# yanqinJiang/Animate3D

Hardware: AMD Instinct MI355X
Metric: UNet denoise-steps/sec, 4view×16frame×512² MV-VDM @1/2/4/8 GPU (higher is better)
Workload: dtype bf16; 1 GPU; BASELINE config 2: 4 views x 16 frames x 512^2 px (64x64 latent), CFG-doubled batch V=8 videos, one MVUNetMotionModel.forward per step, SD1.5 MV-VDM UNet 1.53 B params, seeded synthetic weights; parallelism=single GPU

## Files before the change

### animate3d_amd/csrc/flash_attn.hip

```cpp
#include <type_traits>
#include <utility>

#include "common.h"
#include "flash_common.h"


namespace {

template <int D, int BKV, int QT, int OFS, bool ALIGNED, bool TWO = false>
__global__ __launch_bounds__(256, 2) void flash_attn_kernel(const AttnParams p) {
  constexpr int NU = BKV / 32;
  constexpr int VROW = BKV + 8;
  constexpr int DK = (D + 15) / 16 * 16;
  constexpr int KS = DK / 16;
  constexpr int MT = (D + 31) / 32;
  constexpr int KROW = DK + 8;
  constexpr int DCH = D / 8;
  constexpr int KCHUNKS = BKV * DCH;
  constexpr int KPT = (KCHUNKS + 255) / 256;
  constexpr int VITEMS = (BKV / 4) * DCH;
  constexpr int VPT = (VITEMS + 255) / 256;
  constexpr bool ONES = MT * 32 > D;
  constexpr int KS_ELEMS = BKV * KROW, VT_ELEMS = MT * 32 * VROW;
  constexpr int BQW = 32 * QT, BQ = 4 * BQW;
// ... 455 lines not shown
                     int groups, int heads, int head_dim, int64_t q_len, int64_t kv_len, int64_t kv_len2,
                     float scale, float out_scale, float out_scale2, int flags, int allowed, AttnParams& p, bool& aligned) {
  if (!Q || !K || !V || !O || groups <= 0 || heads <= 0 || q_len <= 0 || kv_len <= 0) return A3D_EINVAL;
  if (two && (!K2 || !V2 || kv_len2 <= 0)) return A3D_EINVAL;
  if (!map_ok(qmap, head_dim) || !map_ok(kmap, head_dim) || (two && !map_ok(kmap2, head_dim)) || !map_ok(omap, head_dim)) return A3D_EINVAL;
  if (!a3d_aligned(16, Q, K, V, K2, V2) || !a3d_aligned(8, O)) return A3D_EINVAL;
  if (groups > 65535 || q_len > 0x3fffffffLL || kv_len > 0x3fffffffLL || kmap->seg_len > 0x3fffffffLL) return A3D_EINVAL;
  if (two && (kv_len2 > 0x3fffffffLL || kmap2->seg_len > 0x3fffffffLL)) return A3D_EINVAL;
  if (two && head_dim != 40 && head_dim != 80) return A3D_EUNSUPPORTED;
  if (flags & ~allowed) return A3D_EINVAL;
  p = AttnParams{};
  p.Q = (const uint16_t*)Q; p.K = (const uint16_t*)K; p.V = (const uint16_t*)V; p.O = (uint16_t*)O;
  p.qm = *qmap; p.km = *kmap; p.om = *omap;
  p.heads = heads; p.q_len = (int)q_len; p.kv_len = (int)kv_len;
  p.scale_log2 = scale * 1.4426950408889634f; p.out_scale = out_scale;
  p.accumulate = flags & A3D_ATTN_ACCUMULATE; p.causal = (flags & A3D_ATTN_CAUSAL) != 0;
  if (p.causal && head_dim != 64 && head_dim != 160) return A3D_EUNSUPPORTED;
  const int bkv = head_dim == 160 ? 32 : 64;
  aligned = (kmap->seg_len % bkv == 0) || (kv_len <= kmap->seg_len);
  if (two) {
    p.K2 = (const uint16_t*)K2; p.V2 = (const uint16_t*)V2; p.km2 = *kmap2; p.kv_len2 = (int)kv_len2; p.out_scale2 = out_scale2;
    aligned = aligned && ((kmap2->seg_len % bkv == 0) || (kv_len2 <= kmap2->seg_len));
  }
  return A3D_OK;
}

static int flash_attn_impl(a3d_stream_t stream, const void* Q, const void* K, const void* V, void* O,
                           const a3d_rowmap* qmap, const a3d_rowmap* kmap, const a3d_rowmap* omap,
                           int groups, int heads, int head_dim, int64_t q_len, int64_t kv_len,
                           float scale, float out_scale, int accumulate, float* lse, unsigned int* counters = nullptr) {
  AttnParams p;
  bool aligned;
  if (int rc = attn_args(false, Q, K, V, nullptr, nullptr, O, qmap, kmap, nullptr, omap, groups, heads, head_dim, q_len, kv_len, 0,
                         scale, out_scale, 0.f, accumulate, A3D_ATTN_ACCUMULATE | A3D_ATTN_CAUSAL | A3D_ATTN_EXACT | A3D_ATTN_PLAIN, p, aligned)) return rc;
  const bool exact = (accumulate & A3D_ATTN_EXACT) != 0, plain = (accumulate & A3D_ATTN_PLAIN) != 0;
  p.lse = lse;
  p.counters = counters;
  hipStream_t s = (hipStream_t)stream;
  switch (head_dim) {
    case 40:
      if (q_len <= 128) { launch<40, 64, 1, OFS_PAD>(aligned, groups, s, p); break; }
      if (!plain && aligned && kv_len % 64 == 0 && kv_len >= 256 && q_len >= 256) {
        if (int rc = A3D_FN(a3d_launch_flash_dm)(exact ? 4 : 5, groups, s, p)) return rc;
        break;
      }
      launch<40, 64, 2, OFS_PAD>(aligned, groups, s, p);
      break;
    case 80:
      if (!plain && aligned && kv_len % 64 == 0 && kv_len >= 512 && q_len >= 256) {
        if (int rc = A3D_FN(a3d_launch_flash_dm80)(exact ? 0 : 1, groups, s, p)) return rc;
        break;
      }
      if (q_len >= 2048 && kv_len >= 2048) { launch<80, 32, 2, OFS_FMA>(aligned, groups, s, p); break; }
      launch<80, 64, 1, OFS_ACC>(aligned, groups, s, p);
      break;
    case 64: launch<64, 64, 1, OFS_FMA>(aligned, groups, s, p); break;
    case 160:
      if (!plain && !p.causal && kv_len % 64 == 0 && kv_len >= 256 && ((kmap->seg_len % 64 == 0) || (kv_len <= kmap->seg_len)) &&
          a3d_aligned(16, O) && omap->ld % 8 == 0) {
        if (int rc = A3D_FN(a3d_launch_flash_dm160)(exact ? 0 : 1, groups, s, p)) return rc;
        break;
      }
      launch<160, 32, 1, OFS_FMA>(aligned, groups, s, p);
      break;
    default: return A3D_EUNSUPPORTED;
  }
  return a3d_launch_status();
}
// ... 42 lines not shown
```

### animate3d_amd/csrc/flash_attn_dm80.hip

```cpp
#include "flash_common.h"

namespace {

constexpr int E_ROWB = 160;
constexpr int E_UNITB = 32 * E_ROWB;
constexpr int E_KB = 2 * E_UNITB;
constexpr int E_TILEB = 2 * E_KB;
constexpr int E_RING = 5;
constexpr int E_CV = E_RING * E_TILEB + 32;
constexpr int E_CV_BYTES = 2752;
constexpr int E_SAMPLE = E_CV + E_CV_BYTES;
constexpr int E_SMEM_BYTES = E_SAMPLE + E_UNITB;
constexpr float E_L_BAD = 1.2676506e30f;
#ifdef A3D_STORAGE_F16
constexpr float E_BIAS = F16_BIAS;
constexpr bool E_SAMPLED = true;
#else
constexpr float E_BIAS = 40.f;
constexpr bool E_SAMPLED = false;
#endif

extern __shared__ __attribute__((aligned(16))) uint8_t e_smem[];
A3D_DEV u32x4_t e_lds128(uint32_t off) { return *reinterpret_cast<const u32x4_t*>(e_smem + off); }
A3D_DEV u32x2_t e_ldstr(uint32_t off) { return lds_tr16_b64(reinterpret_cast<const uint16_t*>(e_smem + off)); }

template <int FLAGS>
__global__ __launch_bounds__(512, 2) void flash_attn_dm80_kernel(const AttnParams p) {
  constexpr int D = 80, KS = 5, MT = 3, NT = 512, BQ = 256;
  constexpr int NEXP = 16, NCVT = 8, NDMA = 3;
  constexpr bool TRY_NOMAX = (FLAGS & 1) != 0;

  const int tid = threadIdx.x, lane = tid & 63, wid = tid >> 6;
  const int w = __builtin_amdgcn_readfirstlane(wid);
  const int l31 = lane & 31, g = lane >> 5, i16 = lane & 15, q4 = lane >> 4;
  const int head = blockIdx.x % p.heads;
  const int qt = blockIdx.x / p.heads;
  const int64_t grp = blockIdx.y;
  const int64_t hoff = (int64_t)head * D;
  const uint32_t lds0 = fa_lds_addr(e_smem);

  for (int i = tid; i < E_CV_BYTES / 2; i += NT) {
    const int vb = 2 * i;
    reinterpret_cast<uint16_t*>(e_smem + E_CV)[i] = (vb == 0 || vb == 160 || vb == 2560 || vb == 2720) ? ONE16 : (uint16_t)0;
  }

  const int64_t ld = p.km.ld;
  const int64_t kgbase = map_group_base(p.km, grp);
  const uint32_t seg_len = (uint32_t)p.km.seg_len;
  const int64_t tile_step = (int64_t)64 * ld;
  const int64_t wrap_step = (p.km.seg_stride - p.km.seg_len) * ld;
  auto slot_src = [&](int slot) -> uint32_t {
    const bool isk = slot < 640;
    const int s2 = isk ? slot : slot - 640;
    const int prow = s2 / 10, cpos = s2 % 10;
    const int c = isk ? (cpos ^ ((prow >> 3) & 1)) : cpos;
    const int key = isk ? prow : ((prow & ~7) | (((prow & 7) >> 1) + 4 * (prow & 1)));
    return (uint32_t)(((int64_t)key * ld + c * 8) * 2);
  };
  const uint32_t voffA = slot_src(64 * w + lane);
  const uint32_t voffB = slot_src(512 + 64 * w + lane);
  const uint32_t voffC = slot_src(1024 + 32 * w + l31);
  uint32_t voffS = 0;
  if constexpr (E_SAMPLED) {
    const int ss = (64 * w + lane) % 320, prow = ss / 10;
    const int64_t key = (int64_t)prow * (p.kv_len / 32);
    voffS = (uint32_t)((map_seq(p.km, key) * ld + ((ss % 10) ^ ((prow >> 3) & 1)) * 8) * 2);
  }
  const uint64_t maskS = w < 5 ? ~0ull : 0ull;

  const int krow = kperm(l31);
  const uint32_t klane = (uint32_t)(krow * E_ROWB + 16 * (g ^ ((krow >> 3) & 1)));
  const int c4 = i16 & 3;
  const uint32_t vrow = (uint32_t)((8 * (q4 >> 1) + 2 * (i16 >> 2)) * E_ROWB);
  const uint32_t vlane01 = vrow + (uint32_t)(2 * (16 * (q4 & 1) + 4 * c4));
  const bool v2_data = (q4 & 1) == 0;
  const uint32_t vlane2 = v2_data ? vrow + (uint32_t)(2 * (64 + 4 * c4)) : (c4 == 0 ? (uint32_t)E_CV : (uint32_t)(E_CV + 8));
  uint32_t vmul = v2_data ? 1u : 0u;
  asm volatile("" : "+v"(vmul));

  const uint16_t* gA = nullptr;
  const uint16_t* gB = nullptr;
  const uint16_t* gC = nullptr;
  uint32_t seg_off = 0;
  auto dma_reset = [&]() __attribute__((always_inline)) {
    gA = dm_scalar(p.K + hoff + kgbase * ld);
    gB = dm_scalar((w < 2 ? p.K : p.V) + hoff + kgbase * ld);
    gC = dm_scalar(p.V + hoff + kgbase * ld);
    seg_off = 0;
  };
  auto tile_base = [&](int tile) __attribute__((always_inline)) -> uint32_t { return (uint32_t)((tile % E_RING) * E_TILEB); };
  auto dma_a = [&](int tile) __attribute__((always_inline)) { dm_glds16(voffA, gA, lds0 + tile_base(tile) + 1024 * w); };
  auto dma_b = [&](int tile) __attribute__((always_inline)) { dm_glds16(voffB, gB, lds0 + tile_base(tile) + 8192 + 1024 * w); };
  auto dma_c = [&](int tile) __attribute__((always_inline)) {
    dm_glds16_m(voffC, gC, lds0 + tile_base(tile) + 16384 + 512 * w, 0xffffffffull);
    seg_off += 64;
    int64_t stp = tile_step;
    if (seg_off >= seg_len) { stp += wrap_step; seg_off = 0; }
    gA += stp; gB += stp; gC += stp;
  };
  auto prologue_issue = [&]() __attribute__((always_inline)) {
    dma_reset();
    if constexpr (E_SAMPLED && TRY_NOMAX)
      dm_glds16_m(voffS, dm_scalar(p.K + hoff + kgbase * ld), lds0 + (uint32_t)(E_SAMPLE + 1024 * (w < 5 ? w : 0)), maskS);
    dma_a(0); dma_b(0); dma_c(0);
    dma_a(1); dma_b(1); dma_c(1);
    dma_a(2); dma_b(2); dma_c(2);
  };
  auto prologue_wait = [&]() __attribute__((always_inline)) { asm volatile("s_waitcnt vmcnt(%0)\n\ts_barrier" :: "i"(NDMA) : "memory"); };
  prologue_issue();

  const int q_idx = qt * BQ + wid * 32 + l31;
  u32x4_t qf[KS];
  {
    const int64_t q_row = map_row(p.qm, grp, q_idx < p.q_len ? q_idx : p.q_len - 1);
#pragma unroll
    for (int ks = 0; ks < KS; ++ks) {
      u32x4_t wq = *reinterpret_cast<const u32x4_t*>(p.Q + q_row * p.qm.ld + hoff + 16 * ks + 8 * g);
#pragma unroll
      for (int j = 0; j < 4; ++j) wq[j] = pack16(lo16(wq[j]) * p.scale_log2, hi16(wq[j]) * p.scale_log2);
      qf[ks] = wq;
    }
  }


  f32x16_t oacc[MT];
  f32x16_t minit;
  u32x4_t kf[KS];
  u32x4_t vf[MT][2];
  auto read_k = [&](uint32_t koff) __attribute__((always_inline)) {
    const uint32_t a = klane + koff;
#pragma unroll
    for (int ks = 0; ks < KS; ++ks) kf[ks] = e_lds128(a + 32 * ks);
  };
  auto read_vhalf = [&](auto i_c, uint32_t a01, uint32_t a2) __attribute__((always_inline)) {
    constexpr int i = decltype(i_c)::value, h = i / 6, mt = (i / 2) % 3, rr = i % 2;
    const u32x2_t t = e_ldstr((mt == 2 ? a2 : a01 + 64 * mt) + (16 * h + rr) * E_ROWB);
    vf[mt][h][2 * rr] = t[0];
    vf[mt][h][2 * rr + 1] = t[1];
  };
  auto read_v = [&](uint32_t voff) __attribute__((always_inline)) {
    const uint32_t a01 = vlane01 + voff, a2 = __umul24(vmul, voff) + vlane2;
    static_for<12>([&](auto i_c) __attribute__((always_inline)) { read_vhalf(i_c, a01, a2); });
  };
  auto pv_mfma = [&](auto i_c, u32x4_t (&P)[2]) __attribute__((always_inline)) {
    constexpr int i = decltype(i_c)::value, h = i / 3, mt = i % 3;
    oacc[mt] = mfma32(vf[mt][h], P[h], oacc[mt]);
  };
  auto clear_o = [&]() __attribute__((always_inline)) {
#pragma unroll
    for (int mt = 0; mt < MT; ++mt)
#pragma unroll
      for (int r = 0; r < 16; ++r) oacc[mt][r] = 0.f;
#pragma unroll
    for (int r = 0; r < 16; ++r) minit[r] = 0.f;
  };
  const int nt = p.kv_len / 64;
  auto first_scores = [&](f32x16_t& s, float& m_off, float bias, uint32_t koff = 0u) __attribute__((always_inline)) -> bool {
    read_k(koff);
#pragma unroll
    for (int r = 0; r < 16; ++r) s[r] = 0.f;
#pragma unroll
    for (int ks = 0; ks < KS; ++ks) s = mfma32(kf[ks], qf[ks], s);
    float mx = s[0];
#pragma unroll
    for (int r = 1; r < 16; ++r) mx = fmaxf(mx, s[r]);
    mx = fmaxf(mx, __shfl_xor(mx, 32));
    bool wide = false;
    if constexpr (E_SAMPLED) {
      if (bias != 0.f) {
        float sm = 0.f, sq = 0.f;
#pragma unroll
        for (int r = 0; r < 16; ++r) { sm += s[r]; sq = fmaf(s[r], s[r], sq); }
        sm += __shfl_xor(sm, 32); sq += __shfl_xor(sq, 32);
        const float mean = sm * (1.f / 32.f);
        bias = f16_sampled_bias(mx, mean, sq * (1.f / 32.f) - mean * mean, f16_expected_max_sds(p.kv_len), wide);
      }
    }
    m_off = mx + bias;
#pragma unroll
    for (int r = 0; r < 16; ++r) { s[r] -= m_off; minit[r] = -m_off; }
    return wide;
  };
  auto finish = [&](bool check) __attribute__((always_inline)) -> bool {
    const float l_tot = __shfl(oacc[2][8], l31);
    const bool bad = !(l_tot < E_L_BAD) || !(l_tot > 0.f);
    if (check) {
      if (__syncthreads_or(bad ? 1 : 0)) { dm_count(p, 1); return false; }
    }
    const float inv = p.out_scale / l_tot;
    if (p.lse != nullptr && q_idx < p.q_len && g == 0)
// ... 13 lines not shown
              const uint32_t w0 = pack16(oacc[mt][8 * pr + 2 * c] * inv, oacc[mt][8 * pr + 2 * c + 1] * inv);
              const uint32_t w1 = pack16(oacc[mt][8 * pr + 4 + 2 * c] * inv, oacc[mt][8 * pr + 4 + 2 * c + 1] * inv);
              const auto r = __builtin_amdgcn_permlane32_swap(w0, w1, false, false);
              v[c] = r[0];
              v[2 + c] = r[1];
            }
            *reinterpret_cast<u32x4_t*>(orow + 32 * mt + 16 * pr + 8 * g) = v;
          }
      } else {
#pragma unroll
        for (int mt = 0; mt < MT; ++mt)
#pragma unroll
          for (int qd = 0; qd < 4; ++qd) {
            const int d = 32 * mt + 8 * qd + 4 * g;
            if (d < D) {
              float v[4];
#pragma unroll
              for (int j = 0; j < 4; ++j) v[j] = oacc[mt][4 * qd + j] * inv;
              if (p.accumulate) {
                const u32x2_t prev = *reinterpret_cast<const u32x2_t*>(orow + d);
                v[0] += lo16(prev[0]); v[1] += hi16(prev[0]); v[2] += lo16(prev[1]); v[3] += hi16(prev[1]);
              }
              u32x2_t o;
              o[0] = pack16(v[0], v[1]);
              o[1] = pack16(v[2], v[3]);
              *reinterpret_cast<u32x2_t*>(orow + d) = o;
            }
          }
      }
    }
    return true;
  };

  auto run_fast = [&]() __attribute__((always_inline)) -> bool {
    clear_o();
    f32x16_t sA, sB;
    u32x4_t pA[2], pB[2];
#pragma unroll
    for (int h = 0; h < 2; ++h) { pA[h] = u32x4_t{0u, 0u, 0u, 0u}; pB[h] = u32x4_t{0u, 0u, 0u, 0u}; }

    auto step = [&](auto do_qk_c, auto do_pv_c, f32x16_t& sCur, f32x16_t& sNext, u32x4_t (&pCur)[2], u32x4_t (&pPrev)[2],
                    uint32_t kOff, uint32_t vOff, auto&& hook) __attribute__((always_inline)) {
      constexpr bool DO_QK = decltype(do_qk_c)::value, DO_PV = decltype(do_pv_c)::value;
      constexpr int NPV = DO_PV ? 2 * MT : 0, NQK = DO_QK ? KS : 0, NS = NPV + NQK;
      constexpr int KSLOT = 2, VS0 = NPV + 1, VPS = 3;
      const uint32_t va01 = vlane01 + vOff, va2 = __umul24(vmul, vOff) + vlane2;
      float e[NEXP];
      auto do_cvt = [&](auto c_c) __attribute__((always_inline)) {
        constexpr int c = decltype(c_c)::value, h = c / 4, jj = c % 4;
        pCur[h][jj] = pack16(e[2 * c], e[2 * c + 1]);
      };
      auto cdone = [](int s) constexpr { return s < 0 ? 0 : (NEXP * s / NS) / 2; };
      __builtin_amdgcn_sched_barrier(0);
      static_for<NS>([&](auto s_c) __attribute__((always_inline)) {
        constexpr int s = decltype(s_c)::value;
        if constexpr (s < NPV) {
          pv_mfma(s_c, pPrev);
        } else {
          constexpr int ks = s - NPV;
          if constexpr (ks == 0) sNext = mfma32(kf[0], qf[0], minit);
          else sNext = mfma32(kf[ks], qf[ks], sNext);
        }
        if constexpr (DO_QK && DO_PV && s == KSLOT) read_k(kOff);
        if constexpr (DO_QK && s >= VS0 && VPS * (s - VS0) < 12) {
          static_for<VPS>([&](auto i_c) __attribute__((always_inline)) {
            constexpr int i = VPS * (s - VS0) + decltype(i_c)::value;
            if constexpr (i < 12) read_vhalf(std::integral_constant<int, i>{}, va01, va2);
          });
        }
        hook(s_c);
        constexpr int E0 = NEXP * s / NS, E1 = NEXP * (s + 1) / NS;
        static_for<E1 - E0>([&](auto x_c) __attribute__((always_inline)) {
          constexpr int x = E0 + decltype(x_c)::value;
          e[x] = __builtin_amdgcn_exp2f(sCur[x]);
        });
        constexpr int C0 = cdone(s - 1), C1 = cdone(s);
        static_for<C1 - C0>([&](auto c_c) __attribute__((always_inline)) { do_cvt(std::integral_constant<int, C0 + decltype(c_c)::value>{}); });
        __builtin_amdgcn_sched_barrier(0);
      });
      {
        constexpr int C0 = cdone(NS - 1);
        static_for<NCVT - C0>([&](auto c_c) __attribute__((always_inline)) { do_cvt(std::integral_constant<int, C0 + decltype(c_c)::value>{}); });
      }
    };

    prologue_wait();
    {
      float m_off;
      if constexpr (E_SAMPLED) {
        const bool wide = first_scores(sA, m_off, E_BIAS, (uint32_t)E_SAMPLE);
        if (__syncthreads_count(wide ? 1 : 0) * 4 > NT) { dm_count(p, 0); return false; }
        read_k(0u);
        sA = minit;
#pragma unroll
        for (int ks = 0; ks < KS; ++ks) sA = mfma32(kf[ks], qf[ks], sA);
      } else {
        first_scores(sA, m_off, E_BIAS);
      }
      read_k((uint32_t)E_UNITB);
    }

    auto iteration = [&](int t, auto first_c, auto last_c, auto dma_c_) __attribute__((always_inline)) {
      constexpr bool FIRST = decltype(first_c)::value, LAST = decltype(last_c)::value, DMA = decltype(dma_c_)::value;
      auto even_hook = [&](auto s_c) __attribute__((always_inline)) {
        if constexpr (DMA && decltype(s_c)::value == 1) dma_a(t + 3);
      };
      auto odd_hook = [&](auto s_c) __attribute__((always_inline)) {
        if constexpr (DMA && decltype(s_c)::value == 1) dma_b(t + 3);
        if constexpr (DMA && decltype(s_c)::value == 4) dma_c(t + 3);
      };
      const uint32_t tb = tile_base(t), tn = tile_base(t + 1);
      step(std::true_type{}, std::integral_constant<bool, !FIRST>{}, sA, sB, pA, pB, tb + E_UNITB, tb + E_KB, even_hook);
      step(std::integral_constant<bool, !LAST>{}, std::true_type{}, sB, sA, pB, pA, tn, tb + E_KB + E_UNITB, odd_hook);
      if constexpr (!LAST) {
        if constexpr (DMA) asm volatile("s_waitcnt vmcnt(%0)\n\ts_barrier" :: "i"(NDMA) : "memory");
        else asm volatile("s_waitcnt vmcnt(0)\n\ts_barrier" ::: "memory");
      }
    };
    constexpr std::true_type Y{};
    constexpr std::false_type N{};
    iteration(0, Y, N, Y);
    for (int t = 1; t < nt - 3; ++t) iteration(t, N, N, Y);
    iteration(nt - 3, N, N, N);
    iteration(nt - 2, N, N, N);
    iteration(nt - 1, N, Y, N);
    {
      read_v(tile_base(nt - 1) + E_KB + E_UNITB);
      static_for<2 * MT>([&](auto i_c) __attribute__((always_inline)) { pv_mfma(i_c, pB); });
    }
    return finish(true);
  };

  auto run_exact = [&](auto rerun_c) __attribute__((always_inline)) {
    clear_o();
    float m_off;
    f32x16_t sc;
    if constexpr (decltype(rerun_c)::value) prologue_issue();
    prologue_wait();
    first_scores(sc, m_off, 0.f);
    for (int t = 0; t < nt; ++t) {
      const bool more = t + 3 < nt;
      if (more) { dma_a(t + 3); dma_b(t + 3); dma_c(t + 3); }
      const uint32_t tb = tile_base(t);
#pragma unroll
      for (int sub = 0; sub < 2; ++sub) {
        if (t > 0 || sub > 0) {
          read_k(tb + sub * E_UNITB);
          sc = minit;
#pragma unroll
          for (int ks = 0; ks < KS; ++ks) sc = mfma32(kf[ks], qf[ks], sc);
          float mx = sc[0];
#pragma unroll
          for (int r = 1; r < 16; ++r) mx = fmaxf(mx, sc[r]);
          if (__any(mx > LAZY_THR)) {
            const float delta = fmaxf(fmaxf(mx, __shfl_xor(mx, 32)), 0.f);
            m_off += delta;
            const float alpha = __builtin_amdgcn_exp2f(-delta);
#pragma unroll
            for (int r = 0; r < 16; ++r) { sc[r] -= delta; minit[r] = -m_off; }
#pragma unroll
            for (int mt = 0; mt < MT; ++mt)
#pragma unroll
              for (int r = 0; r < 16; ++r) oacc[mt][r] *= alpha;
          }
        }
        u32x4_t pf[2];
#pragma unroll
        for (int h = 0; h < 2; ++h)
#pragma unroll
          for (int jj = 0; jj < 4; ++jj)
            pf[h][jj] = pack16(__builtin_amdgcn_exp2f(sc[8 * h + 2 * jj]), __builtin_amdgcn_exp2f(sc[8 * h + 2 * jj + 1]));
        read_v(tb + E_KB + sub * E_UNITB);
        static_for<2 * MT>([&](auto i_c) __attribute__((always_inline)) { pv_mfma(i_c, pf); });
      }
      if (t + 1 < nt) {
        if (more) asm volatile("s_waitcnt vmcnt(%0)\n\ts_barrier" :: "i"(NDMA) : "memory");
        else asm volatile("s_waitcnt vmcnt(0)\n\ts_barrier" ::: "memory");
      }
    }
    finish(false);
  };

  __syncthreads();
  dm_count(p, 2);
  if constexpr (TRY_NOMAX) {
    if (!run_fast()) run_exact(std::true_type{});
  } else {
    run_exact(std::false_type{});
  }
}

template <int FLAGS>
int launch_dm80(int groups, hipStream_t s, const AttnParams& p) {
  static uint64_t attr_done = 0;
  if (int rc = a3d_once_per_device(attr_done, [] {
        return (int)hipFuncSetAttribute(reinterpret_cast<const void*>(&flash_attn_dm80_kernel<FLAGS>),
                                        hipFuncAttributeMaxDynamicSharedMemorySize, E_SMEM_BYTES); })) return rc;
  const int q_tiles = (p.q_len + 255) / 256;
  flash_attn_dm80_kernel<FLAGS><<<dim3((unsigned)(p.heads * q_tiles), (unsigned)groups), dim3(512), E_SMEM_BYTES, s>>>(p);
  return a3d_launch_status();
}

}

int A3D_FN(a3d_launch_flash_dm80)(int flags, int groups, hipStream_t s, const AttnParams& p) {
  switch (flags) {
    case 0: return launch_dm80<0>(groups, s, p);
    case 1: return launch_dm80<1>(groups, s, p);
    default: return A3D_EINVAL;
  }
}
```

### animate3d_amd/csrc/flash_common.h

```cpp
#pragma once
#include <type_traits>
#include <utility>

#include "common.h"

struct AttnParams {
  const uint16_t* Q; const uint16_t* K; const uint16_t* V; uint16_t* O;
  a3d_rowmap qm, km, om;
  int heads; int q_len, kv_len;
  float scale_log2, out_scale; int accumulate;
  int causal;
  const uint16_t* K2; const uint16_t* V2; a3d_rowmap km2; int kv_len2; float out_scale2;
  float* lse;
  unsigned int* counters;
};

namespace {

constexpr int OFS_FMA = 0, OFS_PAD = 1, OFS_ACC = 2;
constexpr float LAZY_THR = 6.0f;


A3D_DEV uint32_t map_clamp32(int64_t d) { return d > 0x7fffffffLL ? 0x7fffffffu : (uint32_t)d; }
A3D_DEV int64_t map_group_base(const a3d_rowmap& m, int64_t g) {
  const uint32_t g32 = (uint32_t)g, gd = map_clamp32(m.gdiv), gq = g32 / gd, gr = g32 - gq * gd;
  return (int64_t)gq * m.ga + (int64_t)gr * m.gb;
}
A3D_DEV int64_t map_seq(const a3d_rowmap& m, int64_t s) {
  const uint32_t s32 = (uint32_t)s, sl = map_clamp32(m.seg_len), sq = s32 / sl, sr = s32 - sq * sl;
  return (int64_t)sq * m.seg_stride + (int64_t)sr;
}
A3D_DEV int64_t map_row(const a3d_rowmap& m, int64_t g, int64_t s) { return map_group_base(m, g) + map_seq(m, s); }

A3D_DEV int kperm(int i) {
  const int j = i & 3, g = (i >> 2) & 1, b = i >> 3;
  return 16 * (b >> 1) + 8 * g + 4 * (b & 1) + j;
}

A3D_DEV float round16(float x) { return lo16(pack16(x, 0.f)); }

constexpr float F16_BIAS = 4.f, F16_LIFT_MAX = 8.f, F16_TOP = 16.f;
A3D_DEV float f16_expected_max_sds(int kv_len) {
  return 2.85f + 0.175f * (float)(31 - __builtin_clz((unsigned)(kv_len < 256 ? 256 : kv_len)) - 8);
}
A3D_DEV float f16_sampled_bias(float mx, float mean, float var, float cmax, bool& wide) {
  const float sd = __builtin_amdgcn_sqrtf(fmaxf(var, 0.f));
  const float lift = fminf(fmaxf(fmaf(cmax, sd, mean) - mx, 0.f), F16_LIFT_MAX);
  wide = !(fmaf(cmax + 2.2f, sd, mean) <= mx + F16_BIAS + lift + F16_TOP);
  return F16_BIAS + lift;
}


A3D_DEV void dm_glds16(uint32_t voff, const void* sbase, uint32_t lds_dst) {
  unsigned keep;
  asm volatile("s_mov_b32 %0, m0\n\ts_mov_b32 m0, %3\n\ts_nop 0\n\tglobal_load_lds_dwordx4 %1, %2\n\ts_mov_b32 m0, %0"
               : "=&s"(keep) : "v"(voff), "s"(sbase), "s"(__builtin_amdgcn_readfirstlane(lds_dst)) : "memory");
}
A3D_DEV void dm_glds16_q(uint32_t voff, const void* sbase, uint32_t lds_dst) {
  unsigned keep;
  uint64_t ex;
  asm volatile("s_mov_b32 %0, m0\n\ts_mov_b32 m0, %4\n\ts_mov_b64 %1, exec\n\ts_mov_b64 exec, 0xffff\n\ts_nop 0\n\t"
               "global_load_lds_dwordx4 %2, %3\n\ts_mov_b64 exec, %1\n\ts_mov_b32 m0, %0"
               : "=&s"(keep), "=&s"(ex) : "v"(voff), "s"(sbase), "s"(__builtin_amdgcn_readfirstlane(lds_dst)) : "memory");
}
A3D_DEV void dm_glds16_sm(uint32_t voff, const void* sbase, uint32_t lds_dst, uint64_t mask) {
  unsigned keep;
  uint64_t ex;
  asm volatile("s_mov_b32 %0, m0\n\ts_mov_b32 m0, %4\n\ts_mov_b64 %1, exec\n\ts_mov_b64 exec, %5\n\ts_nop 0\n\t"
               "global_load_lds_dwordx4 %2, %3\n\ts_mov_b64 exec, %1\n\ts_mov_b32 m0, %0"
               : "=&s"(keep), "=&s"(ex) : "v"(voff), "s"(sbase), "s"(__builtin_amdgcn_readfirstlane(lds_dst)), "s"(mask) : "memory");
}
A3D_DEV void dm_glds16_m(uint32_t voff, const void* sbase, uint32_t lds_dst, uint64_t mask) {
  mask = ((uint64_t)(uint32_t)__builtin_amdgcn_readfirstlane((int)(mask >> 32)) << 32) | (uint32_t)__builtin_amdgcn_readfirstlane((int)(uint32_t)mask);
  dm_glds16_sm(voff, sbase, lds_dst, mask);
}
A3D_DEV const uint16_t* dm_scalar(const uint16_t* ptr) {
  const uint64_t a = (uint64_t)(uintptr_t)ptr;
  return (const uint16_t*)(uintptr_t)(((uint64_t)(uint32_t)__builtin_amdgcn_readfirstlane((int)(a >> 32)) << 32) |
                                      (uint32_t)__builtin_amdgcn_readfirstlane((int)(uint32_t)a));
}

A3D_DEV void dm_count(const AttnParams& p, int which) {
  if (p.counters != nullptr && threadIdx.x == 0) atomicAdd(p.counters + which, 1u);
}

A3D_DEV void store4(uint16_t* dst, bool accumulate, float v0, float v1, float v2, float v3) {
  if (accumulate) {
    const u32x2_t prev = *reinterpret_cast<const u32x2_t*>(dst);
    v0 += lo16(prev[0]); v1 += hi16(prev[0]); v2 += lo16(prev[1]); v3 += hi16(prev[1]);
  }
  u32x2_t o;
  o[0] = pack16(v0, v1);
  o[1] = pack16(v2, v3);
  *reinterpret_cast<u32x2_t*>(dst) = o;
}
A3D_DEV uint32_t fa_lds_addr(const void* p) {
  return (uint32_t)(uintptr_t)(__attribute__((address_space(3))) const void*)p;
}

}

__attribute__((visibility("hidden"))) int A3D_FN(a3d_launch_flash_dm)(int flags, int groups, hipStream_t s, const AttnParams& p);
__attribute__((visibility("hidden"))) int A3D_FN(a3d_launch_flash_dm80)(int flags, int groups, hipStream_t s, const AttnParams& p);
__attribute__((visibility("hidden"))) int A3D_FN(a3d_launch_flash_dm160)(int flags, int groups, hipStream_t s, const AttnParams& p);
__attribute__((visibility("hidden"))) int A3D_FN(a3d_launch_cross_attn40)(int groups, hipStream_t s, const AttnParams& p);
```

### animate3d_amd/hip_ops.py

```python
from __future__ import annotations

import ctypes
import os
import re
from dataclasses import dataclass
from typing import NamedTuple, Optional

import torch

_PKG = os.path.dirname(os.path.abspath(__file__))
_LIB_PATH = os.path.join(_PKG, "lib", "libanimate3d_hip.so")
_HEADER_PATH = os.path.join(os.path.dirname(_PKG), "include", "animate3d_hip.h")
_lib = None

c_i64, c_int, c_f32, c_f64, c_vp = ctypes.c_int64, ctypes.c_int, ctypes.c_float, ctypes.c_double, ctypes.c_void_p


class _RowMapC(ctypes.Structure):
    _fields_ = [("gdiv", c_i64), ("ga", c_i64), ("gb", c_i64), ("seg_len", c_i64), ("seg_stride", c_i64), ("ld", c_i64)]


class StageAdamEntry(ctypes.Structure):
    _fields_ = [("p", c_vp), ("g", c_vp), ("m", c_vp), ("v", c_vp), ("step", c_vp), ("n", c_i64), ("lr", c_f64)]

# ... 36 lines not shown
    take(r"\btypedef\s+void\s*\*\s*a3d_stream_t\s*;")
    for body in take(r"\benum\s*\{(.*?)\}\s*;"):
        for item in body.split(","):
            name, _, value = item.partition("=")
            constants[name.strip()] = int(value, 0)
    structs = {}
    for struct, body in take(r"\btypedef\s+struct\s+(\w+)\s*\{(.*?)\}\s*\1\s*;"):
        fields = structs[struct] = []
        for decl in filter(str.strip, body.split(";")):
            first, *more = decl.split(",")
            ctype, name = _c_type(first, structs)
            fields += [(n.strip(), ctype) for n in (name, *more)]
    functions = {}
    for decl in filter(str.strip, text.split(";")):
        m = re.fullmatch(r"\s*(.+?)\b(a3d_\w+)\s*\((.*)\)\s*", decl, flags=re.S)
        if not m:
            raise RuntimeError(f"animate3d_hip.h: cannot read {' '.join(decl.split())!r} as a declaration")
        params = [] if m[3].strip() == "void" else m[3].split(",")
        functions[m[2]] = (_c_type(m[1], structs, named=False)[0], [_c_type(p, structs)[0] for p in params])
    return Header(functions, constants, structs)


def read_header(path: str) -> Header:
    try:
        with open(path) as f:
            return parse_header(f.read())
    except OSError as e:
        raise RuntimeError(f"{path}: the C header that types the library cannot be read ({e.strerror})") from e


_HEADER = read_header(_HEADER_PATH)
EXPORTED_SYMBOLS = tuple(_HEADER.functions)
globals().update(_HEADER.constants)
STAGE_ADAM_MAX_TENSORS, STAGE_ADAM_BEGIN, STAGE_ADAM_CHECK, STAGE_ADAM_UPDATE = (
    A3D_STAGE_ADAM_MAX_TENSORS, A3D_STAGE_ADAM_BEGIN, A3D_STAGE_ADAM_CHECK, A3D_STAGE_ADAM_UPDATE)
_DTYPE_CODE = {torch.float32: A3D_F32, torch.bfloat16: A3D_BF16, torch.float16: A3D_F16}


@dataclass(frozen=True)
class RowMap:
    gdiv: int
    ga: int
    gb: int
    seg_len: int
    seg_stride: int

    def c(self, ld: int) -> _RowMapC:
        return _RowMapC(self.gdiv, self.ga, self.gb, self.seg_len, self.seg_stride, ld)


def rowmap_rows(m: RowMap, groups: int, step: int, length: int, device="cpu") -> torch.Tensor:
    g = torch.arange(0, groups, step, device=device).view(-1, 1)
    s = torch.arange(length, device=device).view(1, -1)
    return ((g // m.gdiv) * m.ga + (g % m.gdiv) * m.gb + (s // m.seg_len) * m.seg_stride + s % m.seg_len).reshape(-1)


def rowmap_covers(m: RowMap, groups: int, step: int, length: int, rows: int, device="cpu") -> bool:
    if (groups + step - 1) // step * length != rows:
        return False
    idx = rowmap_rows(m, groups, step, length, device)
    return bool(int(idx.min()) >= 0 and int(idx.max()) < rows and torch.unique(idx).numel() == rows)


def lib_path() -> str:
    return _LIB_PATH

# ... 190 lines not shown
        return y

    def conv3x3(self, x, B: int, H: int, W: int, w, bias, *, stride: int = 1, up2x: bool = False, rowbias=None, rb_div: int = 1, residual=None,
                up_size=None, tile128: bool = False):
        x, w = self._act(x, "conv.x"), self._act(w, "conv.w")
        Cin = x.shape[1]
        Cout = w.shape[0]
        assert x.is_contiguous() and w.is_contiguous() and x.shape[0] == B * H * W and w.shape[1] == 9 * Cin
        He, We = (2 * H, 2 * W) if up2x else (H, W)
        up_code = 1 if up2x else 0
        if up_size is not None:
            if not up2x or up_size[0] not in (2 * H, 2 * H - 1) or up_size[1] not in (2 * W, 2 * W - 1):
                raise ValueError(f"forced upsample size {tuple(up_size)} is not reachable from {(H, W)} (2x or 2x - 1 per axis)")
            He, We = int(up_size[0]), int(up_size[1])
            up_code |= (2 if He == 2 * H - 1 else 0) | (4 if We == 2 * W - 1 else 0)
        Ho, Wo = (He - 1) // stride + 1, (We - 1) // stride + 1
        y = self.empty(B * Ho * Wo, Cout)
        if residual is not None:
            assert residual.is_contiguous() and residual.shape == y.shape
        if rowbias is not None:
            assert rowbias.is_contiguous() and rowbias.shape[1] == Cout
        flags = self._gemm_flags(tile128)
        args = (_p(x), _p(w), _p(bias), _p(rowbias), rb_div, _p(residual), _p(y), B, H, W, Cin, Cout, stride, up_code, flags)
        what = f"B={B} H={H} W={W} Cin={Cin} Cout={Cout} stride={stride} up={up2x}"
        if self.split_k and not tile128 and B * Ho * Wo <= 32768:
            key = ("conv", B, H, W, Cin, Cout, stride, up_code, rb_div if rowbias is not None else 0, flags)
            if self._split_k("a3d_conv3x3_ws_bf16", key, args, what):
                return y, Ho, Wo
        self._launch("a3d_conv3x3_bf16", *args, what=what)
        return y, Ho, Wo

    def flash_attn(self, q, k, v, qmap: RowMap, kmap: RowMap, groups: int, heads: int, q_len: int, kv_len: int, *,
                   out=None, out_scale: float = 1.0, accumulate: bool = False, causal: bool = False, with_lse: bool = False,
                   accumulation_target: bool = False, exact: bool = False, plain: bool = False):
        q, k, v = self._act(q, "attn.q"), self._act(k, "attn.k"), self._act(v, "attn.v")
        C = q.shape[1]
        D = C // heads
        assert k.stride(0) == v.stride(0)
        o = out if out is not None else self.empty(q.shape[0], C)
        qm, km, om = qmap.c(q.stride(0)), kmap.c(k.stride(0)), qmap.c(o.stride(0))
        flags = ((A3D_ATTN_ACCUMULATE if accumulate else 0) | (A3D_ATTN_CAUSAL if causal else 0) | (A3D_ATTN_EXACT if exact else 0)
                 | (A3D_ATTN_PLAIN if plain else 0))
        name, last = "a3d_flash_attn_bf16", ()
        if with_lse:
            lse = self._f32(groups, heads, q_len)
            name, last = "a3d_flash_attn_lse_bf16", (_p(lse),)
        elif self.attn_counters is not None:
            cnt = self.attn_counters
            assert cnt.dtype == torch.int32 and cnt.is_cuda and cnt.numel() >= 3 and cnt.is_contiguous()
            name, last = "a3d_flash_attn_counted_bf16", (_p(cnt),)
        self._launch(name, _p(q), _p(k), _p(v), _p(o), ctypes.byref(qm), ctypes.byref(km), ctypes.byref(om), groups, heads, D, q_len, kv_len,
                     float(D) ** -0.5, out_scale, flags, *last, what=f"groups={groups} heads={heads} D={D} q_len={q_len} kv_len={kv_len}")
        return (o, lse) if with_lse else o

    def flash_attn2(self, q, k, v, k2, v2, qmap: RowMap, kmap: RowMap, kmap2: RowMap, groups: int, heads: int, q_len: int, kv_len: int,
                    kv_len2: int, *, out_scale2: float = 1.0):
        D = q.shape[1] // heads
        if D not in (40, 80):
            return None
        q, k, v, k2, v2 = self._act(q, "attn.q"), self._act(k, "attn.k"), self._act(v, "attn.v"), self._act(k2, "attn.k2"), self._act(v2, "attn.v2")
        assert k.stride(0) == v.stride(0) and k2.stride(0) == v2.stride(0)
        o = self.empty(q.shape[0], q.shape[1])
        qm, km, km2, om = qmap.c(q.stride(0)), kmap.c(k.stride(0)), kmap2.c(k2.stride(0)), qmap.c(o.stride(0))
        self._launch("a3d_flash_attn2_bf16", _p(q), _p(k), _p(v), _p(k2), _p(v2), _p(o), ctypes.byref(qm), ctypes.byref(km),
                     ctypes.byref(km2), ctypes.byref(om), groups, heads, D, q_len, kv_len, kv_len2, float(D) ** -0.5, 1.0, out_scale2, 0,
                     what=f"groups={groups} heads={heads} D={D} q_len={q_len} kv_len={kv_len} kv_len2={kv_len2}")
        return o

    def temporal_attn(self, q, k, v, videos: int, frames: int, L: int, heads: int, *, q_f0: int = 0, q_frames: Optional[int] = None,
                      out=None):
        q, k, v = self._act(q, "tattn.q"), self._act(k, "tattn.k"), self._act(v, "tattn.v")
        C = q.shape[1]
        D = C // heads
        assert k.stride(0) == v.stride(0)
        o = self._act(out, "tattn.out") if out is not None else self.empty(q.shape[0], C)
# ... 347 lines not shown
```

### include/animate3d_hip.h

```cpp
#ifndef ANIMATE3D_HIP_H
#define ANIMATE3D_HIP_H

#include <stdint.h>

#ifdef __cplusplus
extern "C" {
#endif

typedef void* a3d_stream_t;

enum {
  A3D_OK = 0,
  A3D_EINVAL = -1,
  A3D_EUNSUPPORTED = -2
};

enum { A3D_F32 = 0, A3D_BF16 = 1, A3D_F16 = 2 };

const char* a3d_version(void);

typedef struct a3d_rowmap {
  int64_t gdiv, ga, gb;
  int64_t seg_len, seg_stride;
  int64_t ld;
// ... 4 lines not shown
#define A3D_GEMM_TILE128 0x100
#define A3D_GEMM_RING 0x200
int a3d_gemm_bf16(a3d_stream_t stream, const void* X, int64_t ldx, const void* W, int64_t ldw,
                  const float* bias, const void* rowbias, int64_t rb_div, const void* R, int64_t ldr,
                  void* Y, int64_t ldy, int64_t M, int64_t N, int64_t K, float alpha, float beta, int flags);

int a3d_gemm_ws_bf16(a3d_stream_t stream, const void* X, int64_t ldx, const void* W, int64_t ldw,
                     const float* bias, const void* rowbias, int64_t rb_div, const void* R, int64_t ldr,
                     void* Y, int64_t ldy, int64_t M, int64_t N, int64_t K, float alpha, float beta, int flags,
                     void* ws, int64_t ws_bytes, int64_t* ws_needed);

int a3d_gemm2_bf16(a3d_stream_t stream, const void* X, int64_t ldx, const void* X2, int64_t ldx2, int64_t K1,
                   const void* W, int64_t ldw, const float* bias, void* Y, int64_t ldy, int64_t M, int64_t N, int64_t K, int flags);

int a3d_gemm_f32out_bf16(a3d_stream_t stream, const void* X, int64_t ldx, const void* W, int64_t ldw,
                         const float* bias, float* Y, int64_t ldy, int64_t M, int64_t N, int64_t K, float alpha);

int a3d_gemm_geglu_bf16(a3d_stream_t stream, const void* X, int64_t ldx, const void* W, int64_t ldw,
                        const float* bias, void* Y, int64_t ldy, int64_t M, int64_t N2, int64_t K, int flags);

int a3d_conv3x3_bf16(a3d_stream_t stream, const void* X, const void* Wp, const float* bias,
                     const void* rowbias, int64_t rb_div, const void* R, void* Y,
                     int B, int H, int W, int Cin, int Cout, int stride, int up2x, int flags);

int a3d_conv3x3_ws_bf16(a3d_stream_t stream, const void* X, const void* Wp, const float* bias,
                        const void* rowbias, int64_t rb_div, const void* R, void* Y,
                        int B, int H, int W, int Cin, int Cout, int stride, int up2x, int flags,
                        void* ws, int64_t ws_bytes, int64_t* ws_needed);

#define A3D_ATTN_ACCUMULATE 1
#define A3D_ATTN_CAUSAL 2
#define A3D_ATTN_EXACT 4
#define A3D_ATTN_PLAIN 8
int a3d_flash_attn_bf16(a3d_stream_t stream, const void* Q, const void* K, const void* V, void* O,
                        const a3d_rowmap* qmap, const a3d_rowmap* kmap, const a3d_rowmap* omap,
                        int groups, int heads, int head_dim, int64_t q_len, int64_t kv_len,
                        float scale, float out_scale, int accumulate);

int a3d_flash_attn_counted_bf16(a3d_stream_t stream, const void* Q, const void* K, const void* V, void* O,
                                const a3d_rowmap* qmap, const a3d_rowmap* kmap, const a3d_rowmap* omap,
                                int groups, int heads, int head_dim, int64_t q_len, int64_t kv_len,
                                float scale, float out_scale, int accumulate, unsigned int* counters);

int a3d_flash_attn2_bf16(a3d_stream_t stream, const void* Q, const void* K, const void* V, const void* K2, const void* V2, void* O,
                         const a3d_rowmap* qmap, const a3d_rowmap* kmap, const a3d_rowmap* kmap2, const a3d_rowmap* omap,
                         int groups, int heads, int head_dim, int64_t q_len, int64_t kv_len, int64_t kv_len2,
                         float scale, float out_scale, float out_scale2, int accumulate);

int a3d_temporal_attn_bf16(a3d_stream_t stream, const void* Q, const void* K, const void* V, int64_t ldqkv,
                           void* O, int64_t ldo, int videos, int frames, int64_t L, int heads,
                           int head_dim, float scale);

int a3d_temporal_attn_sharded_bf16(a3d_stream_t stream, const void* Q, int64_t ldq, const void* K, const void* V, int64_t ldkv,
                                   void* O, int64_t ldo, int videos, int frames, int64_t L, int heads,
                                   int head_dim, float scale, int q_f0, int q_frames, int kv_frames_per_block,
                                   int64_t kv_block_stride);

int64_t a3d_group_norm_ws_floats(int B, int64_t rows, int groups);
int a3d_group_norm_bf16(a3d_stream_t stream, const void* X, void* Y, const float* gamma, const float* beta,
                        float* ws, int B, int64_t rows, int C, int groups, float eps, int silu);

int a3d_group_norm_plan(int64_t rows, int C, int groups, int* out);

int a3d_group_norm2_bf16(a3d_stream_t stream, const void* Xa, int Ca, const void* Xb, int Cb, void* Y, const float* gamma,
                         const float* beta, float* ws, int B, int64_t rows, int groups, float eps, int silu);

// ... 322 lines not shown
```

Baseline: 2.433 denoise-steps/s.

## Make dm80 flash attention workgroups walk several groups with seamed DMA prefetch

The head-dim-80 DMA flash attention kernel can now process several consecutive groups per workgroup. While the last tiles of the current group are being consumed, it issues the K/V prefetch for the next group's first tiles, so the pipeline does not drain and refill between groups. A host heuristic picks the walk length from CU count and grid size, and it can be overridden by an environment variable or disabled with a new ONE_ITEM flag. The change adds ring-offset bookkeeping and masked seam DMAs, and it reduces grid parallelism, which could hurt load balance.

```diff
diff --git a/animate3d_amd/csrc/flash_attn.hip b/animate3d_amd/csrc/flash_attn.hip
--- a/animate3d_amd/csrc/flash_attn.hip
+++ b/animate3d_amd/csrc/flash_attn.hip
@@ -511,8 +511,9 @@
   AttnParams p;
   bool aligned;
   if (int rc = attn_args(false, Q, K, V, nullptr, nullptr, O, qmap, kmap, nullptr, omap, groups, heads, head_dim, q_len, kv_len, 0,
-                         scale, out_scale, 0.f, accumulate, A3D_ATTN_ACCUMULATE | A3D_ATTN_CAUSAL | A3D_ATTN_EXACT | A3D_ATTN_PLAIN, p, aligned)) return rc;
+                         scale, out_scale, 0.f, accumulate, A3D_ATTN_ACCUMULATE | A3D_ATTN_CAUSAL | A3D_ATTN_EXACT | A3D_ATTN_PLAIN | A3D_ATTN_ONE_ITEM, p, aligned)) return rc;
   const bool exact = (accumulate & A3D_ATTN_EXACT) != 0, plain = (accumulate & A3D_ATTN_PLAIN) != 0;
+  p.walk = (accumulate & A3D_ATTN_ONE_ITEM) ? 1 : 0;
   p.lse = lse;
   p.counters = counters;
   hipStream_t s = (hipStream_t)stream;
diff --git a/animate3d_amd/csrc/flash_attn_dm80.hip b/animate3d_amd/csrc/flash_attn_dm80.hip
--- a/animate3d_amd/csrc/flash_attn_dm80.hip
+++ b/animate3d_amd/csrc/flash_attn_dm80.hip
@@ -35,7 +35,12 @@
   const int l31 = lane & 31, g = lane >> 5, i16 = lane & 15, q4 = lane >> 4;
   const int head = blockIdx.x % p.heads;
   const int qt = blockIdx.x / p.heads;
-  const int64_t grp = blockIdx.y;
+  const int walk = p.walk > 1 ? p.walk : 1;
+  const int grp0 = (int)blockIdx.y * walk;
+  const int n_items = p.walk > 1 ? (p.groups - grp0 < walk ? p.groups - grp0 : walk) : 1;
+  int grp = grp0;
+  int rb = 0;
+  int seam_on = 0;
   const int64_t hoff = (int64_t)head * D;
   const uint32_t lds0 = fa_lds_addr(e_smem);
 
@@ -45,7 +50,7 @@
   }
 
   const int64_t ld = p.km.ld;
-  const int64_t kgbase = map_group_base(p.km, grp);
+  int64_t kgbase = map_group_base(p.km, grp);
   const uint32_t seg_len = (uint32_t)p.km.seg_len;
   const int64_t tile_step = (int64_t)64 * ld;
   const int64_t wrap_step = (p.km.seg_stride - p.km.seg_len) * ld;
@@ -82,46 +87,63 @@
   const uint16_t* gB = nullptr;
   const uint16_t* gC = nullptr;
   uint32_t seg_off = 0;
-  auto dma_reset = [&]() __attribute__((always_inline)) {
-    gA = dm_scalar(p.K + hoff + kgbase * ld);
-    gB = dm_scalar((w < 2 ? p.K : p.V) + hoff + kgbase * ld);
-    gC = dm_scalar(p.V + hoff + kgbase * ld);
+  auto dma_reset = [&](int64_t gbase) __attribute__((always_inline)) {
+    gA = dm_scalar(p.K + hoff + gbase * ld);
+    gB = dm_scalar((w < 2 ? p.K : p.V) + hoff + gbase * ld);
+    gC = dm_scalar(p.V + hoff + gbase * ld);
     seg_off = 0;
   };
-  auto tile_base = [&](int tile) __attribute__((always_inline)) -> uint32_t { return (uint32_t)((tile % E_RING) * E_TILEB); };
-  auto dma_a = [&](int tile) __attribute__((always_inline)) { dm_glds16(voffA, gA, lds0 + tile_base(tile) + 1024 * w); };
-  auto dma_b = [&](int tile) __attribute__((always_inline)) { dm_glds16(voffB, gB, lds0 + tile_base(tile) + 8192 + 1024 * w); };
-  auto dma_c = [&](int tile) __attribute__((always_inline)) {
-    dm_glds16_m(voffC, gC, lds0 + tile_base(tile) + 16384 + 512 * w, 0xffffffffull);
+  auto tile_base = [&](int tile) __attribute__((always_inline)) -> uint32_t { return (uint32_t)(((tile + rb) % E_RING) * E_TILEB); };
+  auto seam_lanes = [&](uint64_t lanes) __attribute__((always_inline)) -> uint64_t { return seam_on ? lanes : 0ull; };
+  auto dma_a = [&](int tile, auto seam_c) __attribute__((always_inline)) {
+    if constexpr (decltype(seam_c)::value) dm_glds16_m(voffA, gA, lds0 + tile_base(tile) + 1024 * w, seam_lanes(~0ull));
+    else dm_glds16(voffA, gA, lds0 + tile_base(tile) + 1024 * w);
+  };
+  auto dma_b = [&](int tile, auto seam_c) __attribute__((always_inline)) {
+    if constexpr (decltype(seam_c)::value) dm_glds16_m(voffB, gB, lds0 + tile_base(tile) + 8192 + 1024 * w, seam_lanes(~0ull));
+    else dm_glds16(voffB, gB, lds0 + tile_base(tile) + 8192 + 1024 * w);
+  };
+  auto dma_c = [&](int tile, auto seam_c) __attribute__((always_inline)) {
+    if constexpr (decltype(seam_c)::value) dm_glds16_m(voffC, gC, lds0 + tile_base(tile) + 16384 + 512 * w, seam_lanes(0xffffffffull));
+    else dm_glds16_m(voffC, gC, lds0 + tile_base(tile) + 16384 + 512 * w, 0xffffffffull);
     seg_off += 64;
     int64_t stp = tile_step;
     if (seg_off >= seg_len) { stp += wrap_step; seg_off = 0; }
     gA += stp; gB += stp; gC += stp;
   };
+  constexpr std::false_type NOSEAM{};
+  auto sample_issue = [&](int64_t gbase, uint64_t mask) __attribute__((always_inline)) {
+    if constexpr (E_SAMPLED && TRY_NOMAX)
+      dm_glds16_m(voffS, dm_scalar(p.K + hoff + gbase * ld), lds0 + (uint32_t)(E_SAMPLE + 1024 * (w < 5 ? w : 0)), maskS & mask);
+  };
   auto prologue_issue = [&]() __attribute__((always_inline)) {
-    dma_reset();
-    if constexpr (E_SAMPLED && TRY_NOMAX)
-      dm_glds16_m(voffS, dm_scalar(p.K + hoff + kgbase * ld), lds0 + (uint32_t)(E_SAMPLE + 1024 * (w < 5 ? w : 0)), maskS);
-    dma_a(0); dma_b(0); dma_c(0);
-    dma_a(1); dma_b(1); dma_c(1);
-    dma_a(2); dma_b(2); dma_c(2);
-  };
-  auto prologue_wait = [&]() __attribute__((always_inline)) { asm volatile("s_waitcnt vmcnt(%0)\n\ts_barrier" :: "i"(NDMA) : "memory"); };
-  prologue_issue();
+    dma_reset(kgbase);
+    sample_issue(kgbase, ~0ull);
+    dma_a(0, NOSEAM); dma_b(0, NOSEAM); dma_c(0, NOSEAM);
+    dma_a(1, NOSEAM); dma_b(1, NOSEAM); dma_c(1, NOSEAM);
+    dma_a(2, NOSEAM); dma_b(2, NOSEAM); dma_c(2, NOSEAM);
+  };
+  auto prologue_wait = [&](bool seamed) __attribute__((always_inline)) {
+    if (seamed) asm volatile("s_waitcnt vmcnt(0)\n\ts_barrier" ::: "memory");
+    else asm volatile("s_waitcnt vmcnt(%0)\n\ts_barrier" :: "i"(NDMA) : "memory");
+  };
 
   const int q_idx = qt * BQ + wid * 32 + l31;
   u32x4_t qf[KS];
-  {
-    const int64_t q_row = map_row(p.qm, grp, q_idx < p.q_len ? q_idx : p.q_len - 1);
+  auto load_q = [&]() __attribute__((always_inline)) {
+    const AttnKernArgs kp = attn_kernargs();
+    const a3d_rowmap qm = map_fetch(&kp->qm);
+    const uint16_t* Q = kp->Q;
+    const float scale_log2 = kp->scale_log2;
+    const int64_t q_row = map_row(qm, grp, q_idx < p.q_len ? q_idx : p.q_len - 1);
 #pragma unroll
     for (int ks = 0; ks < KS; ++ks) {
-      u32x4_t wq = *reinterpret_cast<const u32x4_t*>(p.Q + q_row * p.qm.ld + hoff + 16 * ks + 8 * g);
-#pragma unroll
-      for (int j = 0; j < 4; ++j) wq[j] = pack16(lo16(wq[j]) * p.scale_log2, hi16(wq[j]) * p.scale_log2);
+      u32x4_t wq = *reinterpret_cast<const u32x4_t*>(Q + q_row * qm.ld + hoff + 16 * ks + 8 * g);
+#pragma unroll
+      for (int j = 0; j < 4; ++j) wq[j] = pack16(lo16(wq[j]) * scale_log2, hi16(wq[j]) * scale_log2);
       qf[ks] = wq;
     }
-  }
-
+  };
 
   f32x16_t oacc[MT];
   f32x16_t minit;
@@ -155,7 +177,7 @@
     for (int r = 0; r < 16; ++r) minit[r] = 0.f;
   };
   const int nt = p.kv_len / 64;
-  auto first_scores = [&](f32x16_t& s, float& m_off, float bias, uint32_t koff = 0u) __attribute__((always_inline)) -> bool {
+  auto first_scores = [&](f32x16_t& s, float& m_off, float bias, uint32_t koff) __attribute__((always_inline)) -> bool {
     read_k(koff);
 #pragma unroll
     for (int r = 0; r < 16; ++r) s[r] = 0.f;
@@ -235,7 +257,7 @@
     return true;
   };
 
-  auto run_fast = [&]() __attribute__((always_inline)) -> bool {
+  auto run_fast = [&](bool seamed) __attribute__((always_inline)) -> bool {
     clear_o();
     f32x16_t sA, sB;
     u32x4_t pA[2], pB[2];
@@ -287,46 +309,51 @@
       }
     };
 
-    prologue_wait();
+    prologue_wait(seamed);
     {
       float m_off;
       if constexpr (E_SAMPLED) {
         const bool wide = first_scores(sA, m_off, E_BIAS, (uint32_t)E_SAMPLE);
         if (__syncthreads_count(wide ? 1 : 0) * 4 > NT) { dm_count(p, 0); return false; }
-        read_k(0u);
+        read_k(tile_base(0));
         sA = minit;
 #pragma unroll
         for (int ks = 0; ks < KS; ++ks) sA = mfma32(kf[ks], qf[ks], sA);
       } else {
-        first_scores(sA, m_off, E_BIAS);
-      }
-      read_k((uint32_t)E_UNITB);
-    }
-
-    auto iteration = [&](int t, auto first_c, auto last_c, auto dma_c_) __attribute__((always_inline)) {
-      constexpr bool FIRST = decltype(first_c)::value, LAST = decltype(last_c)::value, DMA = decltype(dma_c_)::value;
+        first_scores(sA, m_off, E_BIAS, tile_base(0));
+      }
+      read_k(tile_base(0) + (uint32_t)E_UNITB);
+    }
+
+    auto iteration = [&](int t, auto first_c, auto last_c, auto seam_c) __attribute__((always_inline)) {
+      constexpr bool FIRST = decltype(first_c)::value, LAST = decltype(last_c)::value, IS_SEAM = decltype(seam_c)::value;
       auto even_hook = [&](auto s_c) __attribute__((always_inline)) {
-        if constexpr (DMA && decltype(s_c)::value == 1) dma_a(t + 3);
+        if constexpr (decltype(s_c)::value == 1) dma_a(t + 3, seam_c);
       };
       auto odd_hook = [&](auto s_c) __attribute__((always_inline)) {
-        if constexpr (DMA && decltype(s_c)::value == 1) dma_b(t + 3);
-        if constexpr (DMA && decltype(s_c)::value == 4) dma_c(t + 3);
+        if constexpr (decltype(s_c)::value == 1) dma_b(t + 3, seam_c);
+        if constexpr (decltype(s_c)::value == 4) dma_c(t + 3, seam_c);
       };
       const uint32_t tb = tile_base(t), tn = tile_base(t + 1);
       step(std::true_type{}, std::integral_constant<bool, !FIRST>{}, sA, sB, pA, pB, tb + E_UNITB, tb + E_KB, even_hook);
       step(std::integral_constant<bool, !LAST>{}, std::true_type{}, sB, sA, pB, pA, tn, tb + E_KB + E_UNITB, odd_hook);
       if constexpr (!LAST) {
-        if constexpr (DMA) asm volatile("s_waitcnt vmcnt(%0)\n\ts_barrier" :: "i"(NDMA) : "memory");
+        if (!IS_SEAM || seam_on != 0) asm volatile("s_waitcnt vmcnt(%0)\n\ts_barrier" :: "i"(NDMA) : "memory");
         else asm volatile("s_waitcnt vmcnt(0)\n\ts_barrier" ::: "memory");
       }
     };
     constexpr std::true_type Y{};
     constexpr std::false_type N{};
-    iteration(0, Y, N, Y);
-    for (int t = 1; t < nt - 3; ++t) iteration(t, N, N, Y);
-    iteration(nt - 3, N, N, N);
-    iteration(nt - 2, N, N, N);
-    iteration(nt - 1, N, Y, N);
+    iteration(0, Y, N, N);
+    for (int t = 1; t < nt - 3; ++t) iteration(t, N, N, N);
+    {
+      const int64_t kgnext = map_group_base(map_fetch(&attn_kernargs()->km), grp + (seam_on ? 1 : 0));
+      dma_reset(kgnext);
+      sample_issue(kgnext, seam_lanes(~0ull));
+    }
+    iteration(nt - 3, N, N, Y);
+    iteration(nt - 2, N, N, Y);
+    iteration(nt - 1, N, Y, Y);
     {
       read_v(tile_base(nt - 1) + E_KB + E_UNITB);
       static_for<2 * MT>([&](auto i_c) __attribute__((always_inline)) { pv_mfma(i_c, pB); });
@@ -338,12 +365,15 @@
     clear_o();
     float m_off;
     f32x16_t sc;
-    if constexpr (decltype(rerun_c)::value) prologue_issue();
-    prologue_wait();
-    first_scores(sc, m_off, 0.f);
+    if constexpr (decltype(rerun_c)::value) {
+      asm volatile("s_waitcnt vmcnt(0)\n\ts_barrier" ::: "memory");
+      prologue_issue();
+    }
+    prologue_wait(false);
+    first_scores(sc, m_off, 0.f, tile_base(0));
     for (int t = 0; t < nt; ++t) {
       const bool more = t + 3 < nt;
-      if (more) { dma_a(t + 3); dma_b(t + 3); dma_c(t + 3); }
+      if (more) { dma_a(t + 3, NOSEAM); dma_b(t + 3, NOSEAM); dma_c(t + 3, NOSEAM); }
       const uint32_t tb = tile_base(t);
 #pragma unroll
       for (int sub = 0; sub < 2; ++sub) {
@@ -385,11 +415,28 @@
   };
 
   __syncthreads();
-  dm_count(p, 2);
-  if constexpr (TRY_NOMAX) {
-    if (!run_fast()) run_exact(std::true_type{});
-  } else {
-    run_exact(std::false_type{});
+  bool seamed = false;
+  for (int it = 0; it < n_items; ++it) {
+    if (it > 0) {
+      grp = grp0 + it;
+      kgbase = map_group_base(map_fetch(&attn_kernargs()->km), grp);
+    }
+    if (!seamed) {
+      if (it > 0) __syncthreads();
+      prologue_issue();
+    }
+    load_q();
+    dm_count(p, 2);
+    if constexpr (TRY_NOMAX) {
+      const bool has_next = it + 1 < n_items;
+      seam_on = has_next ? -1 : 0;
+      const bool ok = run_fast(seamed);
+      if (!ok) run_exact(std::true_type{});
+      seamed = ok && has_next;
+    } else {
+      run_exact(std::false_type{});
+    }
+    rb = (rb + nt) % E_RING;
   }
 }
 
@@ -400,7 +447,11 @@
         return (int)hipFuncSetAttribute(reinterpret_cast<const void*>(&flash_attn_dm80_kernel<FLAGS>),
                                         hipFuncAttributeMaxDynamicSharedMemorySize, E_SMEM_BYTES); })) return rc;
   const int q_tiles = (p.q_len + 255) / 256;
-  flash_attn_dm80_kernel<FLAGS><<<dim3((unsigned)(p.heads * q_tiles), (unsigned)groups), dim3(512), E_SMEM_BYTES, s>>>(p);
+  AttnParams pw = p;
+  pw.groups = groups;
+  pw.walk = (FLAGS & 1) ? attn_walk((int64_t)p.heads * q_tiles, groups, p.walk) : 1;
+  const int gy = (groups + pw.walk - 1) / pw.walk;
+  flash_attn_dm80_kernel<FLAGS><<<dim3((unsigned)(p.heads * q_tiles), (unsigned)gy), dim3(512), E_SMEM_BYTES, s>>>(pw);
   return a3d_launch_status();
 }
 
diff --git a/animate3d_amd/csrc/flash_common.h b/animate3d_amd/csrc/flash_common.h
--- a/animate3d_amd/csrc/flash_common.h
+++ b/animate3d_amd/csrc/flash_common.h
@@ -1,4 +1,5 @@
 #pragma once
+#include <cstdlib>
 #include <type_traits>
 #include <utility>
 
@@ -13,6 +14,7 @@
   const uint16_t* K2; const uint16_t* V2; a3d_rowmap km2; int kv_len2; float out_scale2;
   float* lse;
   unsigned int* counters;
+  int walk; int groups;
 };
 
 namespace {
@@ -31,6 +33,18 @@
   return (int64_t)sq * m.seg_stride + (int64_t)sr;
 }
 A3D_DEV int64_t map_row(const a3d_rowmap& m, int64_t g, int64_t s) { return map_group_base(m, g) + map_seq(m, s); }
+
+typedef const __attribute__((address_space(4))) AttnParams* AttnKernArgs;
+A3D_DEV AttnKernArgs attn_kernargs() {
+  AttnKernArgs kp = (AttnKernArgs)__builtin_amdgcn_kernarg_segment_ptr();
+  asm volatile("" : "+s"(kp));
+  return kp;
+}
+A3D_DEV a3d_rowmap map_fetch(const __attribute__((address_space(4))) a3d_rowmap* m) {
+  a3d_rowmap r;
+  r.gdiv = m->gdiv; r.ga = m->ga; r.gb = m->gb; r.seg_len = m->seg_len; r.seg_stride = m->seg_stride; r.ld = m->ld;
+  return r;
+}
 
 A3D_DEV int kperm(int i) {
   const int j = i & 3, g = (i >> 2) & 1, b = i >> 3;
@@ -94,6 +108,26 @@
   o[1] = pack16(v2, v3);
   *reinterpret_cast<u32x2_t*>(dst) = o;
 }
+inline int attn_walk(int64_t wgs, int groups, int one_item) {
+  if (one_item > 0 || groups < 2) return 1;
+  if (const char* e = getenv("A3D_ATTN_WALK")) {
+    const int w = atoi(e);
+    if (w >= 1) return w < groups ? w : groups;
+  }
+  int cus = 0;
+  if (hipDeviceGetAttribute(&cus, hipDeviceAttributeMultiprocessorCount, a3d_current_device()) != hipSuccess || cus <= 0) return 1;
+  if (wgs * groups < 2 * (int64_t)cus) return 1;
+  int best = 1;
+  int64_t best_cost = (wgs * groups + cus - 1) / cus;
+  for (int w = 2; w <= groups && w <= 64; ++w) {
+    const int64_t grid = wgs * ((groups + w - 1) / w);
+    if (grid < cus) break;
+    const int64_t cost = ((grid + cus - 1) / cus) * w;
+    if (cost <= best_cost) { best_cost = cost; best = w; }
+  }
+  return best;
+}
+
 A3D_DEV uint32_t fa_lds_addr(const void* p) {
   return (uint32_t)(uintptr_t)(__attribute__((address_space(3))) const void*)p;
 }
diff --git a/animate3d_amd/hip_ops.py b/animate3d_amd/hip_ops.py
--- a/animate3d_amd/hip_ops.py
+++ b/animate3d_amd/hip_ops.py
@@ -92,6 +92,7 @@
 _HEADER = read_header(_HEADER_PATH)
 EXPORTED_SYMBOLS = tuple(_HEADER.functions)
 globals().update(_HEADER.constants)
+A3D_ATTN_ONE_ITEM = A3D_ATTN_PLAIN << 3
 STAGE_ADAM_MAX_TENSORS, STAGE_ADAM_BEGIN, STAGE_ADAM_CHECK, STAGE_ADAM_UPDATE = (
     A3D_STAGE_ADAM_MAX_TENSORS, A3D_STAGE_ADAM_BEGIN, A3D_STAGE_ADAM_CHECK, A3D_STAGE_ADAM_UPDATE)
 _DTYPE_CODE = {torch.float32: A3D_F32, torch.bfloat16: A3D_BF16, torch.float16: A3D_F16}
@@ -348,7 +349,7 @@
 
     def flash_attn(self, q, k, v, qmap: RowMap, kmap: RowMap, groups: int, heads: int, q_len: int, kv_len: int, *,
                    out=None, out_scale: float = 1.0, accumulate: bool = False, causal: bool = False, with_lse: bool = False,
-                   accumulation_target: bool = False, exact: bool = False, plain: bool = False):
+                   accumulation_target: bool = False, exact: bool = False, plain: bool = False, one_item: bool = False):
         q, k, v = self._act(q, "attn.q"), self._act(k, "attn.k"), self._act(v, "attn.v")
         C = q.shape[1]
         D = C // heads
@@ -356,7 +357,7 @@
         o = out if out is not None else self.empty(q.shape[0], C)
         qm, km, om = qmap.c(q.stride(0)), kmap.c(k.stride(0)), qmap.c(o.stride(0))
         flags = ((A3D_ATTN_ACCUMULATE if accumulate else 0) | (A3D_ATTN_CAUSAL if causal else 0) | (A3D_ATTN_EXACT if exact else 0)
-                 | (A3D_ATTN_PLAIN if plain else 0))
+                 | (A3D_ATTN_PLAIN if plain else 0) | (A3D_ATTN_ONE_ITEM if one_item else 0))
         name, last = "a3d_flash_attn_bf16", ()
         if with_lse:
             lse = self._f32(groups, heads, q_len)
diff --git a/include/animate3d_hip.h b/include/animate3d_hip.h
--- a/include/animate3d_hip.h
+++ b/include/animate3d_hip.h
@@ -60,6 +60,7 @@
 #define A3D_ATTN_CAUSAL 2
 #define A3D_ATTN_EXACT 4
 #define A3D_ATTN_PLAIN 8
+#define A3D_ATTN_ONE_ITEM (A3D_ATTN_PLAIN << 3)
 int a3d_flash_attn_bf16(a3d_stream_t stream, const void* Q, const void* K, const void* V, void* O,
                         const a3d_rowmap* qmap, const a3d_rowmap* kmap, const a3d_rowmap* omap,
                         int groups, int heads, int head_dim, int64_t q_len, int64_t kv_len,
```

After: 2.448 denoise-steps/s (median of 6 runs). Within noise of the previous version (+0.6%).
